# myfavouritekk/vdetlib

Measured on AMD Instinct MI355X. Metric: boxes/sec whole-node (NMS+temporal-conv+link), 300f×10k-box synth; mAP parity, higher is better.
Workload: dtype f32; 1 GPU; configs[1]+[2]: 1 video/GPU, 300 frames x 10000 boxes x 200 classes; per-(frame,class) NMS thresh 0.30 + temporal max-pool w=3 + 3-tap temporal convolution; greedy tubelets: 10 tracks/class (stop < 0.90), IoU-link >= 0.50, spatial max-pool IoU > 0.70 + completion + temporal max-pool; frames=300, boxes=10000, classes=200, scores=rand, parallelism=video-per-gpu x1, 4 distinct videos in flight per GPU

## Files before the change

### vdetlib_amd/csrc/nms_kernels.hpp

```cpp
#pragma once
#include <hip/hip_runtime.h>
#include <stdint.h>

namespace vdet {

struct GroupDesc {
    int32_t box_off;
    int32_t nbox;
    int64_t bits_off;
};

__device__ __host__ __forceinline__ int64_t bit_word(int nbox, int v, int c)
{
    const int W = (nbox + 63) >> 6;
    return ((int64_t)(v >> 6) * W + c) * 64 + (v & 63);
}
__host__ __device__ __forceinline__ int64_t bit_words_of_group(int nbox)
{
    const int64_t W = (nbox + 63) >> 6;
    return W * W * 64;
}

struct TileDesc {
    int32_t group;
// ... 870 lines not shown
        for (int i = tid; i < NW * 256; i += BLOCK) bases[i] = 0;
        __syncthreads();
        uint32_t ra[CPW];
        uint32_t rl[CPW];
        bool peel_on = false;
#pragma unroll
        for (int ch = 0; ch < CPW; ++ch) {
            const int q = (c0 + ch) * 64 + lane;
            const bool valid = (c0 + ch) < nchunks && q < N;
            const uint32_t i = valid ? src[q] : 0u;
            const uint32_t d = valid ? (((uint32_t)keys0[i] >> shift) & 255u) : 0u;
            ra[ch] = i | (d << 16);
            if (ARANK) {
                uint32_t r = 0u;
                bool pending = valid;
#pragma unroll
                for (int peel = 0; peel < 2; ++peel) {
                    if (ch > 0 && !peel_on) break;
                    const unsigned long long rem = __ballot(pending);
                    if (rem) {
                        const int l0 = __ffsll((unsigned long long)rem) - 1;
                        const uint32_t d0 = (uint32_t)__builtin_amdgcn_readlane((int)d, l0);
                        const bool mine = pending && d == d0;
                        const unsigned long long m = __ballot(mine);
                        if (ch == 0 && peel == 0) peel_on = (pass == 3) || __popcll(m) >= 12;
                        if (peel_on) {
                            const uint32_t rank = __builtin_amdgcn_mbcnt_hi((uint32_t)(m >> 32), __builtin_amdgcn_mbcnt_lo((uint32_t)m, 0u));
                            uint32_t old = 0u;
                            if (lane == l0) old = atomicAdd(&bases[w * 256 + d0], (uint32_t)__popcll(m));
                            old = (uint32_t)__builtin_amdgcn_readlane((int)old, l0);
                            if (mine) { r = old + rank; pending = false; }
                        } else {
                            break;
                        }
                    }
                }
                if (pending) r = atomicAdd(&bases[w * 256 + d], 1u);
                rl[ch] = r;
            } else {
                const unsigned long long peers = match8(d, valid);
                const uint32_t rank = __builtin_amdgcn_mbcnt_hi((uint32_t)(peers >> 32), __builtin_amdgcn_mbcnt_lo((uint32_t)peers, 0u));
                uint32_t old = 0;
                if (valid && rank == 0) old = atomicAdd(&bases[w * 256 + d], (uint32_t)__popcll(peers));
                const int leader = valid ? (__ffsll((unsigned long long)peers) - 1) : lane;
                old = __shfl(old, leader, 64);
                rl[ch] = old + rank;
            }
        }
        __syncthreads();
        uint32_t dsum = 0, dincl = 0;
        if (tid < 256) {
#pragma unroll
            for (int ww = 0; ww < NW; ++ww) dsum += bases[ww * 256 + tid];
            dincl = dsum;
#define VDET_SCAN_STEP(CTRL, ROWMASK) dincl += (uint32_t)__builtin_amdgcn_update_dpp(0, (int)dincl, CTRL, ROWMASK, 0xf, false);
            VDET_SCAN_STEP(0x111, 0xf) VDET_SCAN_STEP(0x112, 0xf) VDET_SCAN_STEP(0x114, 0xf) VDET_SCAN_STEP(0x118, 0xf)
            VDET_SCAN_STEP(0x142, 0xa) VDET_SCAN_STEP(0x143, 0xc)
#undef VDET_SCAN_STEP
            if (lane == 63) swt[w] = dincl;
        }
        __syncthreads();
        if (tid < 256) {
            uint32_t run = dincl - dsum;
            for (int k = 0; k < w; ++k) run += swt[k];
#pragma unroll
            for (int ww = 0; ww < NW; ++ww) {
                const uint32_t c = bases[ww * 256 + tid];
                bases[ww * 256 + tid] = run;
                run += c;
            }
        }
        __syncthreads();
#pragma unroll
        for (int ch = 0; ch < CPW; ++ch) {
            const int q = (c0 + ch) * 64 + lane;
            const bool valid = (c0 + ch) < nchunks && q < N;
            if (valid) {
                const uint32_t d = ra[ch] >> 16;
                dst[bases[w * 256 + d] + rl[ch]] = (uint16_t)(ra[ch] & 0xFFFFu);
            }
        }
        __syncthreads();
        uint16_t *t = src; src = dst; dst = t;
    }
    int ncand_out = ncand;
    if (prm.topk > 0 && ncand > prm.topk) {
        const int k = prm.topk;
        if (w == 0) {
            auto key_at = [&](int q) -> uint32_t {
                const int i = src[q];
                if (prm.keys) return prm.keys[pr.sbase + i];
                return score_key(prm.scores[pr.sbase + (int64_t)i * pr.sstride]);
            };
            const uint32_t kk = key_at(k - 1);
            int a = k - 1, b = k;
            for (;;) {
                const int q = a - 1 - lane;
                const bool eq = q >= 0 && key_at(q) == kk;
                const unsigned long long m = __ballot(eq);
                const int n = m == ~0ull ? 64 : (__ffsll((unsigned long long)~m) - 1);
                a -= n;
                if (n < 64) break;
            }
            for (;;) {
                const int q = b + lane;
                const bool eq = q < ncand && key_at(q) == kk;
                const unsigned long long m = __ballot(eq);
                const int n = m == ~0ull ? 64 : (__ffsll((unsigned long long)~m) - 1);
                b += n;
                if (n < 64) break;
            }
            const int nsel = k - a, s0 = b - nsel;
            if (s0 > a)
                for (int t = 0; t < nsel; t += 64) {
                    const bool v = t + lane < nsel;
                    const uint16_t e = v ? src[s0 + t + lane] : (uint16_t)0;
                    __builtin_amdgcn_fence(__ATOMIC_ACQ_REL, "wavefront");
                    if (v) src[a + t + lane] = e;
                    __builtin_amdgcn_fence(__ATOMIC_ACQ_REL, "wavefront");
                }
        }
        ncand_out = k;
        __syncthreads();
    }
    uint16_t *out = prm.order + pr.obase;
    if (((pr.obase | (int64_t)N) & 1) == 0) {
        uint32_t *out2 = reinterpret_cast<uint32_t *>(out);
        const uint32_t *src2 = reinterpret_cast<const uint32_t *>(src);
        for (int v = tid; v < (N >> 1); v += BLOCK) out2[v] = src2[v];
    } else {
        for (int v = tid; v < N; v += BLOCK) out[v] = src[v];
    }
    if (tid == 0) {
        prm.ncand[p] = ncand_out;
        if (prm.nover) prm.nover[p] = ncand;
    }
}

template <int BLOCK, int CPW, bool ARANK>
__global__ __launch_bounds__(BLOCK, (BLOCK == 1024 && CPW <= 10) ? 8 : 1) void sort_kernel(const SortParams prm)
{
    extern __shared__ __attribute__((aligned(16))) unsigned char smem[];
    const int p = xcd_problem(blockIdx.x, gridDim.x);
    if (p >= prm.P) return;
    lsd_sort_problem<BLOCK, CPW, ARANK>(prm, p, smem);
}

template <int BLOCK, int CPW, bool ARANK>
__global__ __launch_bounds__(BLOCK, (BLOCK == 1024 && CPW <= 10) ? 8 : 1) void sort_list_kernel(const SortParams prm, const int32_t *__restrict__ list,
                                                                                                   const int *__restrict__ count)
{
    extern __shared__ __attribute__((aligned(16))) unsigned char smem[];
    const int n = *count;
    for (int i = blockIdx.x; i < n; i += gridDim.x) {
        lsd_sort_problem<BLOCK, CPW, ARANK>(prm, list[i], smem);
        __syncthreads();
    }
}

__global__ __launch_bounds__(64) void lds_atomic_order_probe(const uint8_t *__restrict__ pats, int n, int *__restrict__ bad)
{
    __shared__ uint32_t tbl[256];
    const int lane = threadIdx.x;
    int nbad = 0;
    for (int t = blockIdx.x; t < n; t += gridDim.x) {
        for (int i = lane; i < 256; i += 64) tbl[i] = 0;
        __builtin_amdgcn_fence(__ATOMIC_ACQ_REL, "wavefront");
        const uint32_t d = pats[t * 64 + lane];
        const bool act = d != 255;
        uint32_t r1 = 0, r2 = 0;
        if (act) r1 = atomicAdd(&tbl[d], 1u);
        if (act) r2 = atomicAdd(&tbl[d], 1u);
        const unsigned long long peers = match8(d, act);
        const uint32_t rank = __builtin_amdgcn_mbcnt_hi((uint32_t)(peers >> 32), __builtin_amdgcn_mbcnt_lo((uint32_t)peers, 0u));
        const uint32_t cnt = (uint32_t)__popcll(peers);
        if (act && (r1 != rank || r2 != cnt + rank)) nbad = 1;
        __builtin_amdgcn_fence(__ATOMIC_ACQ_REL, "wavefront");
    }
    if (__ballot(nbad) && lane == 0) atomicOr(bad, 1);
}

__global__ __launch_bounds__(256) void transpose_keys_kernel(const float *__restrict__ scores, uint32_t *__restrict__ keys,
                                                             int B, int C, int use_thr, float thr)
{
    __shared__ uint32_t tile[64][65];
    const int f = blockIdx.z;
    const int b0 = blockIdx.x * 64, c0 = blockIdx.y * 64;
    const int tx = threadIdx.x & 63, ty = threadIdx.x >> 6;
    const float *src = scores + (int64_t)f * B * C;
    for (int r = ty; r < 64; r += 4) {
        const int b = b0 + r, c = c0 + tx;
        uint32_t k = 0;
        if (b < B && c < C) {
            const float s = src[(int64_t)b * C + c];
            k = score_key(s);
            if (use_thr && !(s > thr)) k = 0u;
        }
        tile[r][tx] = k;
    }
    __syncthreads();
    uint32_t *dst = keys + (int64_t)f * C * B;
    for (int r = ty; r < 64; r += 4) {
        const int c = c0 + r, b = b0 + tx;
        if (c < C && b < B) dst[(int64_t)c * B + b] = tile[tx][r];
    }
}

struct WalkParams {
    int mode, P, B, C;
    const GroupDesc *groups;
    const uint16_t *order;
    const int32_t *ncand;
    const uint2 *row_meta;
    const uint16_t *adj;
    const uint32_t *group_z;
    int32_t *keep_idx;
    int32_t *keep_cnt;
    int64_t cap;
    int *status;
    int mask_words;
    const uint32_t *group_flags;
    int wave_words;
    int packed;
    const WalkMeta *wmeta;
    float t32;
    int adj32;
    const uint4 *wmeta16;
};

typedef __attribute__((address_space(3))) uint32_t lds_u32_t;
typedef volatile lds_u32_t *lds_mask_t;

__device__ __forceinline__ lds_mask_t lds_mask_ptr(unsigned char *dyn_smem, int word_off)
{
    return (lds_mask_t)((__attribute__((address_space(3))) unsigned char *)dyn_smem) + word_off;
}
__device__ __forceinline__ void lds_or(lds_mask_t m, int word, uint32_t bits)
{
    __hip_atomic_fetch_or((lds_u32_t *)(m + word), bits, __ATOMIC_RELAXED, __HIP_MEMORY_SCOPE_WAVEFRONT);
}
__device__ __forceinline__ void lds_and(lds_mask_t m, int word, uint32_t bits)
{
    __hip_atomic_fetch_and((lds_u32_t *)(m + word), bits, __ATOMIC_RELAXED, __HIP_MEMORY_SCOPE_WAVEFRONT);
}

__device__ __forceinline__ void lds_or_pair(lds_mask_t m, uint32_t d)
{
    uint32_t w0, w1;
    asm("v_bfe_u32 %0, %1, 5, 11" : "=v"(w0) : "v"(d));
    asm("v_bfe_u32 %0, %1, 21, 11" : "=v"(w1) : "v"(d));
    lds_or(m, (int)w0, 1u << (d & 31u));
    lds_or(m, (int)w1, 1u << ((d >> 16) & 31u));
}

constexpr int kWalkGrp = 4;

template <bool HASZ>
__device__ __forceinline__ void walk_apply_slice(lds_mask_t mask, uint16_t e, bool in_range, int &bad)
{
    if (HASZ) {
        if (in_range) {
            const int v = e & 0x7FFF;
            if (e & kZTag) { if (!((mask[v >> 5] >> (v & 31)) & 1u)) bad = 1; }
            else lds_or(mask, v >> 5, 1u << (v & 31));
        }
    } else {
        if (in_range) lds_or(mask, e >> 5, 1u << (e & 31));
    }
}

template <bool HASZ>
__device__ __forceinline__ void walk_group(lds_mask_t mask, const uint16_t *__restrict__ adj, int lane, int c,
                                           uint32_t off, int deg, const int (&ls)[kWalkGrp], int ng,
                                           const uint32_t (&pre)[kWalkGrp], unsigned long long &kept_lanes, int &bad)
{
#pragma unroll
    for (int k = 0; k < kWalkGrp; ++k) {
        if (k >= ng) break;
        const int cu = __builtin_amdgcn_readlane(c, ls[k]);
        if (__builtin_amdgcn_readfirstlane((mask[cu >> 5] >> (cu & 31)) & 1u)) continue;
        kept_lanes |= 1ull << ls[k];
        const int d = __builtin_amdgcn_readlane(deg, ls[k]);
        if (HASZ && lane == 0) lds_or(mask, cu >> 5, 1u << (cu & 31));
        if (2 * lane < d) {
            walk_apply_slice<HASZ>(mask, (uint16_t)(pre[k] & 0xFFFFu), true, bad);
            walk_apply_slice<HASZ>(mask, (uint16_t)(pre[k] >> 16), true, bad);
        }
        if (d > 128) {
            const uint32_t o = __builtin_amdgcn_readlane(off, ls[k]);
            for (int e0 = 128; e0 < d; e0 += 64)
                walk_apply_slice<HASZ>(mask, adj[o + min(e0 + lane, d - 1)], e0 + lane < d, bad);
        }
    }
}


constexpr int kPackRing = 72;
struct __attribute__((aligned(16))) AdjVec { uint32_t v[4]; };
typedef float lds_f4v __attribute__((ext_vector_type(4)));
typedef volatile __attribute__((address_space(3))) lds_f4v *lds_f4_t;

__device__ __forceinline__ int ring_wrap(int s) { return s >= kPackRing ? s - kPackRing : s; }

__device__ __forceinline__ void walk_ring_drain(const WalkParams &prm, lds_mask_t mask, lds_mask_t ring, lds_f4_t ringb, const int lane,
                                                const float t32, const bool flush, int &qh, int &qn, int &nk,
                                                int32_t *__restrict__ out, const int64_t cap)
{
    const int k = lane >> 3, sub = lane & 7;
    while (qn >= 8 || (flush && qn > 0)) {
        const int ng = min(8, qn);
        const int s = ring_wrap(qh + k);
        const bool vk = k < ng;
        const int sj = ring_wrap(qh + sub);
        const lds_f4v mi = ringb[2 * s];
        const int cm = vk ? (int)__float_as_uint(mi.x) : 0;
        const lds_f4v vi = ringb[2 * s + 1], vj = ringb[2 * sj + 1];
        const float4 bi = make_float4(vi.x, vi.y, vi.z, vi.w), bj = make_float4(vj.x, vj.y, vj.z, vj.w);
        const bool live = vk && !((mask[cm >> 5] >> (cm & 31)) & 1u);
        const unsigned long long lm = __ballot(live);
        const float ai = mi.w, aj = __uint_as_float(ring[8 * sj + 3]);
        bool border;
        bool hit = pred_regular(bi, ai, bj, aj, t32, t32 * 4.76837158203125e-7f, border);
        if (__ballot(border) != 0ull) {
            if (border) hit = (pair_pred(bi, ai, bj, aj, t32) & 1u) != 0u;
        }
        const unsigned long long cmask = __ballot(hit && k < sub && sub < ng && live && ((lm >> (8 * sub)) & 1ull));
        unsigned long long surv_s = lm & 0x0101010101010101ull;
        if (cmask) {
            unsigned long long sv = 0ull;
            for (int j = 0; j < 8; ++j) {
                const unsigned long long col = (cmask >> j) & 0x0101010101010101ull;
                if (((lm >> (8 * j)) & 1ull) && !(col & sv)) sv |= 1ull << (8 * j);
            }
            surv_s = sv;
        }
        const bool surv = (surv_s >> (lane & 56)) & 1ull;
        if (surv_s) {
            const int pos = nk + (int)__builtin_amdgcn_mbcnt_hi((uint32_t)(surv_s >> 32),
                                                               __builtin_amdgcn_mbcnt_lo((uint32_t)surv_s, 0u));
            if (surv && sub == 0 && (int64_t)pos < cap) out[(uint32_t)pos] = cm;
            nk += __popcll(surv_s);
            const uint32_t off = surv ? __float_as_uint(mi.y) : 0u;
            const int deg = surv ? (int)__float_as_uint(mi.z) : 0;
            AdjVec a0, a1;
            if (prm.adj32) {
                const uint32_t bo = off * 2u;
                const char *ab = reinterpret_cast<const char *>(prm.adj);
                a0 = *reinterpret_cast<const AdjVec *>(ab + (bo + (8 * sub < deg ? 16u * (uint32_t)sub : 0u)));
                a1 = *reinterpret_cast<const AdjVec *>(ab + (bo + (64 + 8 * sub < deg ? 128u + 16u * (uint32_t)sub : 0u)));
            } else {
                const AdjVec *pa = reinterpret_cast<const AdjVec *>(prm.adj + off);
                a0 = pa[8 * sub < deg ? sub : 0];
                a1 = pa[64 + 8 * sub < deg ? 8 + sub : 0];
            }
            const bool has0 = 8 * sub < deg, has1 = 64 + 8 * sub < deg;
            if (has0) {
#pragma unroll
                for (int t = 0; t < 4; ++t) {
                    const uint32_t d = a0.v[t];
                    lds_or_pair(mask, d);
                }
            }
            if (__ballot(has1) != 0ull) {
                if (has1) {
#pragma unroll
                    for (int t = 0; t < 4; ++t) {
                        const uint32_t d = a1.v[t];
                        lds_or_pair(mask, d);
                    }
                }
                unsigned long long lg = __ballot(sub == 0 && deg > 128);
                while (lg) {
                    const int l = __ffsll((unsigned long long)lg) - 1;
                    lg &= lg - 1;
                    const uint32_t o = __builtin_amdgcn_readlane(off, l);
                    const int dl = __builtin_amdgcn_readlane(deg, l);
                    for (int e0 = 128; e0 < dl; e0 += 64) {
                        const uint32_t e = prm.adj[o + min(e0 + lane, dl - 1)];
                        if (e0 + lane < dl) lds_or(mask, (int)(e >> 5), 1u << (e & 31u));
                    }
                }
            }
            __builtin_amdgcn_s_waitcnt(0x0F70);
        }
        qh = ring_wrap(qh + ng);
        qn -= ng;
    }
}

template <bool U16>
__device__ __forceinline__ void walk_list_packed(const WalkParams &prm, lds_mask_t mask, const int lane, const int rb,
                                                 const uint16_t *__restrict__ order, const int ncand,
                                                 int32_t *__restrict__ out, const int64_t cap, int &nk_out)
{
    lds_mask_t ring = mask + prm.mask_words;
    lds_f4_t ringb = (lds_f4_t)ring;
    const WalkMeta *__restrict__ wmeta = prm.wmeta + rb;
    const uint4 *__restrict__ wm16 = U16 ? prm.wmeta16 + rb : nullptr;
    const float t32 = prm.t32;
    int qh = 0, qn = 0, nk = 0;
    const int last = max(ncand - 1, 0);
    int cc[3];
    uint2 mm[3];
    float4 bb[3];
    uint4 rr[3];
    cc[0] = (int)order[(uint32_t)min(lane, last)];
    cc[1] = (int)order[(uint32_t)min(64 + lane, last)];
    cc[2] = 0;
    mm[0] = mm[1] = mm[2] = make_uint2(0u, 0u);
    bb[0] = bb[1] = bb[2] = make_float4(0.f, 0.f, 0.f, 0.f);
    rr[0] = rr[1] = rr[2] = make_uint4(0u, 0u, 0u, 0u);
    if (lane < ncand) {
        if (U16) rr[0] = wm16[(uint32_t)cc[0]];
        else { const WalkMeta *wm = wmeta + (uint32_t)cc[0]; bb[0] = wm->box; const uint4 rw = wm->row; mm[0] = make_uint2(rw.x, rw.y); }
    }
#define VDET_WALK_PASS(Q0, CUR, NXT, NN)                                                                                             \
    {                                                                                                                                \
        const int q0_ = (Q0);                                                                                                        \
        const int c = cc[CUR];                                                                                                       \
        cc[NN] = (int)order[(uint32_t)min(q0_ + 128 + lane, last)];                                                                  \
        {    \
             \
            const bool want = (q0_ + 64 + lane) < ncand && !((mask[cc[NXT] >> 5] >> (cc[NXT] & 31)) & 1u);                           \
            if (U16) rr[NXT] = wm16[want ? (uint32_t)cc[NXT] : 0u];                                                                  \
            else {                                                                                                                   \
                const WalkMeta *wm = wmeta + (want ? (uint32_t)cc[NXT] : 0u);                                                        \
                bb[NXT] = wm->box; const uint4 rw = wm->row; mm[NXT] = make_uint2(rw.x, rw.y);                                       \
            }                                                                                                                        \
        }                                                                                                                            \
        const bool alive = (q0_ + lane) < ncand && !((mask[c >> 5] >> (c & 31)) & 1u);                                               \
        const unsigned long long am = __ballot(alive);                                                                               \
        if (alive) {                                                                                                                 \
            const int s = ring_wrap(qh + qn + (int)__builtin_amdgcn_mbcnt_hi((uint32_t)(am >> 32), __builtin_amdgcn_mbcnt_lo((uint32_t)am, 0u))); \
            ring[8 * s] = (uint32_t)c;                                                                                               \
            lds_f4v bv;                                                                                                              \
            if (U16) {                                                                                                               \
                ring[8 * s + 1] = rr[CUR].z;                                                                                         \
                ring[8 * s + 2] = rr[CUR].w;                                                                                         \
                bv.x = (float)(rr[CUR].x & 0xFFFFu); bv.y = (float)(rr[CUR].x >> 16);                                                \
                bv.z = (float)(rr[CUR].y & 0xFFFFu); bv.w = (float)(rr[CUR].y >> 16);                                                \
            } else {                                                                                                                 \
                ring[8 * s + 1] = mm[CUR].x;                                                                                         \
                ring[8 * s + 2] = mm[CUR].y;                                                                                         \
                bv.x = bb[CUR].x; bv.y = bb[CUR].y; bv.z = bb[CUR].z; bv.w = bb[CUR].w;                                              \
            }                                                                                                                        \
            ringb[2 * s + 1] = bv;                                                                                                   \
            ring[8 * s + 3] = __float_as_uint(box_area(make_float4(bv.x, bv.y, bv.z, bv.w)));                                        \
        }                                                                                                                            \
        qn += __popcll(am);                                                                                                          \
        walk_ring_drain(prm, mask, ring, ringb, lane, t32, q0_ + 64 >= ncand, qh, qn, nk, out, cap);                                 \
    }
    for (int q0 = 0; q0 < ncand; q0 += 192) {
        VDET_WALK_PASS(q0, 0, 1, 2)
        if (q0 + 64 >= ncand) break;
        VDET_WALK_PASS(q0 + 64, 1, 2, 0)
        if (q0 + 128 >= ncand) break;
        VDET_WALK_PASS(q0 + 128, 2, 0, 1)
    }
#undef VDET_WALK_PASS
    nk_out = nk;
}

__device__ __forceinline__ void walk_one(const WalkParams &prm, const int p, unsigned char *smem, const int lane, const int w)
{
    lds_mask_t mask = lds_mask_ptr(smem, w * prm.wave_words);
    const ProblemRef pr = decode_problem(prm.mode, p, prm.B, prm.C, prm.groups);
    const int N = pr.N, rb = pr.rb;
    const uint16_t *order = prm.order + pr.obase;
    const int ncand = prm.ncand[p];
    const bool has_z = prm.group_z[pr.g] != 0;
    const bool regular = !has_z && prm.group_flags && (prm.group_flags[pr.g] & kFlagRegular);
    int32_t *out = prm.keep_idx + (prm.mode == 2 ? (int64_t)rb : (int64_t)p * prm.cap);
    const int64_t cap = prm.mode == 2 ? (int64_t)N : prm.cap;

    for (int i = lane; i < ((N + 31) >> 5); i += 64) mask[i] = 0u;
    __builtin_amdgcn_fence(__ATOMIC_ACQ_REL, "wavefront");
    if (has_z) {
        for (int q = ncand + lane; q < N; q += 64) {
            const int v = order[q];
            lds_or(mask, v >> 5, 1u << (v & 31));
        }
        __builtin_amdgcn_fence(__ATOMIC_ACQ_REL, "wavefront");
    }

    int nk = 0;
    int bad = 0;
    if (regular && prm.packed && N >= 2) {
        if (prm.wmeta16 && (prm.group_flags[pr.g] & kFlagU16)) walk_list_packed<true>(prm, mask, lane, rb, order, ncand, out, cap, nk);
        else walk_list_packed<false>(prm, mask, lane, rb, order, ncand, out, cap, nk);
        if (lane == 0) prm.keep_cnt[p] = nk;
        if ((int64_t)nk > cap && lane == 0) atomicOr(prm.status, kStCap);
        return;
    }
    const uint32_t *adjw = reinterpret_cast<const uint32_t *>(prm.adj);
    const int last = max(ncand - 1, 0);
    int c_cur = (int)order[min(lane, last)];
    int c_nxt = (int)order[min(64 + lane, last)];
    uint2 m_cur = make_uint2(0u, 0u);
    if (lane < ncand) m_cur = prm.row_meta[rb + c_cur];
    for (int q0 = 0; q0 < ncand; q0 += 64) {
        const int q = q0 + lane;
        const bool valid = q < ncand;
        const int c = c_cur;
        const int c_nn = (int)order[min(q0 + 128 + lane, last)];
        uint2 m_nxt = make_uint2(0u, 0u);
        if ((q + 64) < ncand && !((mask[c_nxt >> 5] >> (c_nxt & 31)) & 1u)) m_nxt = prm.row_meta[rb + c_nxt];
        const bool alive = valid && !((mask[c >> 5] >> (c & 31)) & 1u);
        unsigned long long am = __ballot(alive);
        unsigned long long kept_lanes = 0ull;
        const uint32_t off = m_cur.x;
        const int deg = (int)m_cur.y;
        while (am) {
            int ls[kWalkGrp];
            int ng = 0;
#pragma unroll
            for (int k = 0; k < kWalkGrp; ++k) {
                ls[k] = k ? ls[k - 1] : 0;
                if (am) { ls[k] = __builtin_amdgcn_readfirstlane(__ffsll((unsigned long long)am) - 1); am &= am - 1; ng = k + 1; }
            }
            uint32_t pre[kWalkGrp];
#pragma unroll
            for (int k = 0; k < kWalkGrp; ++k) {
                const uint32_t o = __builtin_amdgcn_readlane(off, ls[k]);
                const int d = __builtin_amdgcn_readlane(deg, ls[k]);
                pre[k] = adjw[(o >> 1) + min(lane, (max(d, 1) - 1) >> 1)];
            }
            if (has_z) walk_group<true>(mask, prm.adj, lane, c, off, deg, ls, ng, pre, kept_lanes, bad);
            else walk_group<false>(mask, prm.adj, lane, c, off, deg, ls, ng, pre, kept_lanes, bad);
        }
        if (kept_lanes) {
            const int pos = nk + (int)__builtin_amdgcn_mbcnt_hi((uint32_t)(kept_lanes >> 32),
                                                               __builtin_amdgcn_mbcnt_lo((uint32_t)kept_lanes, 0u));
            if (((kept_lanes >> lane) & 1ull) && (int64_t)pos < cap) out[pos] = c;
            nk += __popcll(kept_lanes);
        }
        c_cur = c_nxt; c_nxt = c_nn; m_cur = m_nxt;
    }
    if (lane == 0) prm.keep_cnt[p] = nk;
    if ((int64_t)nk > cap && lane == 0) atomicOr(prm.status, kStCap);
    if (__ballot(bad != 0) && lane == 0) atomicOr(prm.status, kStDivZero);
}

__global__ __launch_bounds__(256) void walk_kernel(const WalkParams prm)
{
    extern __shared__ __attribute__((aligned(16))) unsigned char smem[];
    const int lane = threadIdx.x & 63, w = __builtin_amdgcn_readfirstlane(threadIdx.x >> 6);
    const int nwaves_total = gridDim.x * 4;
    const int per = nwaves_total >> 3;
    const int p = (blockIdx.x & 7) * per + (blockIdx.x >> 3) * 4 + w;
    if (p >= prm.P) return;
    walk_one(prm, p, smem, lane, w);
}

__global__ __launch_bounds__(256) void check_order_kernel(const uint16_t *__restrict__ order, const int32_t *__restrict__ ncand_in, int P, int B,
                                                          int32_t *__restrict__ ncand_out, int *__restrict__ status)
{
    const int lane = threadIdx.x & 63;
    const int p = blockIdx.x * 4 + (threadIdx.x >> 6);
    if (p >= P) return;
    const int n = ncand_in[p];
    bool bad = n < 0 || n > B;
    if (!bad)
        for (int q = lane; q < n; q += 64) bad = bad || (int)order[(int64_t)p * B + q] >= B;
    const bool any = __ballot(bad) != 0ull;
    if (lane == 0) {
        ncand_out[p] = any ? 0 : n;
        if (any) atomicOr(status, kStBadOrder);
    }
}

__global__ __launch_bounds__(256) void gather_comp_kernel(const GroupDesc *__restrict__ groups, int P,
                                                          const int32_t *__restrict__ keep_idx,
                                                          const int32_t *__restrict__ keep_cnt,
                                                          const float *__restrict__ scores,
                                                          const uint32_t *__restrict__ keys,
                                                          const uint32_t *__restrict__ orig_idx,
                                                          unsigned long long *__restrict__ comp,
                                                          unsigned int *__restrict__ glob_cnt)
{
    __shared__ unsigned int sbase;
    const int p = blockIdx.x;
    if (p >= P) return;
    const int rb = groups[p].box_off;
    const int K = keep_cnt[p];
    if (threadIdx.x == 0) sbase = atomicAdd(glob_cnt, (unsigned int)K);
    __syncthreads();
    const unsigned int base = sbase;
    for (int k = threadIdx.x; k < K; k += 256) {
        const int v = keep_idx[rb + k];
        const uint32_t key = keys ? keys[rb + v] : score_key(scores[rb + v]);
        comp[base + k] = ((unsigned long long)key << 32) | orig_idx[rb + v];
    }
}

__global__ void bitonic_global_step(unsigned long long *__restrict__ data, uint32_t n2, uint32_t j, uint32_t k)
{
    const uint32_t i = blockIdx.x * blockDim.x + threadIdx.x;
    if (i >= n2) return;
    const uint32_t ixj = i ^ j;
    if (ixj > i) {
        const unsigned long long a = data[i], b = data[ixj];
        const bool desc = (i & k) == 0;
        if (desc ? (a < b) : (a > b)) { data[i] = b; data[ixj] = a; }
    }
}

__global__ __launch_bounds__(1024) void bitonic_lds_kernel(unsigned long long *__restrict__ data, uint32_t n2,
                                                           uint32_t k_first, uint32_t k_last)
{
    __shared__ unsigned long long s[2048];
    const uint32_t base = blockIdx.x * 2048u;
    const uint32_t tid = threadIdx.x;
    for (uint32_t i = tid; i < 2048u; i += 1024u) s[i] = (base + i < n2) ? data[base + i] : 0ull;
    __syncthreads();
    for (uint32_t k = k_first; k <= k_last; k <<= 1) {
        uint32_t j0 = k >> 1;
        if (j0 > 1024u) j0 = 1024u;
        for (uint32_t j = j0; j > 0; j >>= 1) {
            for (uint32_t li = tid; li < 2048u; li += 1024u) {
                const uint32_t lixj = li ^ j;
                if (lixj > li) {
                    const uint32_t gi = base + li;
                    const unsigned long long a = s[li], b = s[lixj];
                    const bool desc = (gi & k) == 0;
                    if (desc ? (a < b) : (a > b)) { s[li] = b; s[lixj] = a; }
                }
            }
            __syncthreads();
        }
    }
    for (uint32_t i = tid; i < 2048u; i += 1024u)
        if (base + i < n2) data[base + i] = s[i];
}

__global__ void fill_comp_kernel(const float *__restrict__ scores, const uint32_t *__restrict__ keys,
                                 const uint8_t *__restrict__ excl, int use_thr, float thr, int64_t base, int n,
                                 uint32_t n2, unsigned long long *__restrict__ comp, int32_t *__restrict__ ncand_p)
{
    const uint32_t i = blockIdx.x * blockDim.x + threadIdx.x;
    if (i >= n2) return;
    unsigned long long c = 0ull;
    if ((int)i < n) {
        uint32_t k;
        bool x = false;
        if (keys) { k = keys[base + i]; x = (k == 0u); }
        else {
            const float sc = scores[base + i];
            k = score_key(sc);
            if (use_thr && !(sc > thr)) x = true;
        }
        if (excl && excl[base + i]) x = true;
        if (x) k = 0u; else atomicAdd(ncand_p, 1);
        c = ((unsigned long long)k << 32) | i;
    }
    comp[i] = c;
}

__global__ void comp_to_order_kernel(const unsigned long long *__restrict__ comp, int n, uint16_t *__restrict__ order)
{
    const int i = blockIdx.x * blockDim.x + threadIdx.x;
    if (i < n) order[i] = (uint16_t)(comp[i] & 0xFFFFull);
}

__global__ void comp_to_index_kernel(const unsigned long long *__restrict__ comp, uint32_t n, int64_t *__restrict__ out)
{
    const uint32_t i = blockIdx.x * blockDim.x + threadIdx.x;
    if (i < n) out[i] = (int64_t)(comp[i] & 0xFFFFFFFFull);
}

__global__ void track_round1_kernel(const float *__restrict__ det_frame, const float4 *__restrict__ det_box, int m,
                                    const float *__restrict__ trk_frame, const float4 *__restrict__ trk_box, int t,
                                    float t32, uint8_t *__restrict__ excl, int *__restrict__ status)
{
    const int i = blockIdx.x * blockDim.x + threadIdx.x;
    if (i >= m) return;
    const float4 bi = det_box[i];
    const float iarea = box_area(bi);
    const float fi = det_frame[i];
    uint8_t sup = 0;
    for (int j = 0; j < t; ++j) {
        if (fi != trk_frame[j]) continue;
        const float4 bt = trk_box[j];
        const uint32_t p = pair_pred(bi, iarea, bt, box_area(bt), t32);
        if (p & 2u) { atomicOr(status, kStDivZero); break; }
        if (p & 1u) { sup = 1; break; }
    }
    excl[i] = sup;
}

}
```

Before: 348.2 million boxes/s.

## Software-pipeline adjacency list loads across ring-drain groups in NMS walk

Restructures the NMS walk's ring drain so the adjacency vectors for the next 8-candidate group are requested before the current group's suppression bits are applied. Partial waitcnts then overlap the global-memory latency with the LDS mask OR work. The kept-index write becomes a branchless raw buffer store, with out-of-range offsets used to drop masked lanes. The walk kernel also gets an 8-waves-per-EU occupancy hint. In exchange, adjacency rows are loaded for groups whose candidates may not survive, and the forced occupancy may push the kernel into register spills.

```diff
diff --git a/vdetlib_amd/csrc/nms_kernels.hpp b/vdetlib_amd/csrc/nms_kernels.hpp
--- a/vdetlib_amd/csrc/nms_kernels.hpp
+++ b/vdetlib_amd/csrc/nms_kernels.hpp
@@ -1196,90 +1196,122 @@
 
 __device__ __forceinline__ int ring_wrap(int s) { return s >= kPackRing ? s - kPackRing : s; }
 
+__device__ __forceinline__ void walk_lists_request(const WalkParams &prm, lds_f4_t ringb, const int qh, const int ng, const int k,
+                                                   const int sub, AdjVec &a0, AdjVec &a1)
+{
+    const lds_f4v mi = ringb[2 * ring_wrap(qh + k)];
+    const bool vk = k < ng;
+    const uint32_t off = vk ? __float_as_uint(mi.y) : 0u;
+    const int deg = vk ? (int)__float_as_uint(mi.z) : 0;
+    if (prm.adj32) {
+        const uint32_t bo = off * 2u;
+        const char *ab = reinterpret_cast<const char *>(prm.adj);
+        a0 = *reinterpret_cast<const AdjVec *>(ab + (bo + (8 * sub < deg ? 16u * (uint32_t)sub : 0u)));
+        a1 = *reinterpret_cast<const AdjVec *>(ab + (bo + (64 + 8 * sub < deg ? 128u + 16u * (uint32_t)sub : 0u)));
+    } else {
+        const AdjVec *pa = reinterpret_cast<const AdjVec *>(prm.adj + off);
+        a0 = pa[8 * sub < deg ? sub : 0];
+        a1 = pa[64 + 8 * sub < deg ? 8 + sub : 0];
+    }
+}
+
+__device__ __forceinline__ unsigned long long walk_group_survivors(lds_mask_t mask, lds_mask_t ring, lds_f4_t ringb, const int qh, const int ng,
+                                                                   const int k, const int sub, const float t32, int &cm, uint32_t &off, int &deg)
+{
+    const int s = ring_wrap(qh + k);
+    const bool vk = k < ng;
+    const int sj = ring_wrap(qh + sub);
+    const lds_f4v mi = ringb[2 * s];
+    cm = vk ? (int)__float_as_uint(mi.x) : 0;
+    off = __float_as_uint(mi.y);
+    deg = (int)__float_as_uint(mi.z);
+    const lds_f4v vi = ringb[2 * s + 1], vj = ringb[2 * sj + 1];
+    const float4 bi = make_float4(vi.x, vi.y, vi.z, vi.w), bj = make_float4(vj.x, vj.y, vj.z, vj.w);
+    const bool live = vk && !((mask[cm >> 5] >> (cm & 31)) & 1u);
+    const unsigned long long lm = __ballot(live);
+    const float ai = mi.w, aj = __uint_as_float(ring[8 * sj + 3]);
+    bool border;
+    bool hit = pred_regular(bi, ai, bj, aj, t32, t32 * 4.76837158203125e-7f, border);
+    if (__ballot(border) != 0ull) {
+        if (border) hit = (pair_pred(bi, ai, bj, aj, t32) & 1u) != 0u;
+    }
+    const unsigned long long cmask = __ballot(hit && k < sub && sub < ng && live && ((lm >> (8 * sub)) & 1ull));
+    unsigned long long surv_s = lm & 0x0101010101010101ull;
+    if (cmask) {
+        unsigned long long sv = 0ull;
+        for (int j = 0; j < 8; ++j) {
+            const unsigned long long col = (cmask >> j) & 0x0101010101010101ull;
+            if (((lm >> (8 * j)) & 1ull) && !(col & sv)) sv |= 1ull << (8 * j);
+        }
+        surv_s = sv;
+    }
+    return surv_s;
+}
+
+__device__ __forceinline__ void walk_lists_apply(const WalkParams &prm, lds_mask_t mask, const int lane, const int sub, const bool surv,
+                                                 const uint32_t off, const int deg, const AdjVec &a0, const AdjVec &a1)
+{
+    const bool has0 = surv && 8 * sub < deg, has1 = surv && 64 + 8 * sub < deg;
+    if (has0) {
+#pragma unroll
+        for (int t = 0; t < 4; ++t) {
+            const uint32_t d = a0.v[t];
+            lds_or_pair(mask, d);
+        }
+    }
+    if (__ballot(has1) != 0ull) {
+        if (has1) {
+#pragma unroll
+            for (int t = 0; t < 4; ++t) {
+                const uint32_t d = a1.v[t];
+                lds_or_pair(mask, d);
+            }
+        }
+        unsigned long long lg = __ballot(surv && sub == 0 && deg > 128);
+        while (lg) {
+            const int l = __ffsll((unsigned long long)lg) - 1;
+            lg &= lg - 1;
+            const uint32_t o = __builtin_amdgcn_readlane(off, l);
+            const int dl = __builtin_amdgcn_readlane(deg, l);
+            for (int e0 = 128; e0 < dl; e0 += 64) {
+                const uint32_t e = prm.adj[o + min(e0 + lane, dl - 1)];
+                if (e0 + lane < dl) lds_or(mask, (int)(e >> 5), 1u << (e & 31u));
+            }
+        }
+    }
+}
+
 __device__ __forceinline__ void walk_ring_drain(const WalkParams &prm, lds_mask_t mask, lds_mask_t ring, lds_f4_t ringb, const int lane,
                                                 const float t32, const bool flush, int &qh, int &qn, int &nk,
-                                                int32_t *__restrict__ out, const int64_t cap)
+                                                const __amdgpu_buffer_rsrc_t outr, const int64_t cap)
 {
     const int k = lane >> 3, sub = lane & 7;
-    while (qn >= 8 || (flush && qn > 0)) {
+    auto turn = [&](const AdjVec &c0, const AdjVec &c1, AdjVec &n0, AdjVec &n1) __attribute__((always_inline)) -> bool {
         const int ng = min(8, qn);
-        const int s = ring_wrap(qh + k);
-        const bool vk = k < ng;
-        const int sj = ring_wrap(qh + sub);
-        const lds_f4v mi = ringb[2 * s];
-        const int cm = vk ? (int)__float_as_uint(mi.x) : 0;
-        const lds_f4v vi = ringb[2 * s + 1], vj = ringb[2 * sj + 1];
-        const float4 bi = make_float4(vi.x, vi.y, vi.z, vi.w), bj = make_float4(vj.x, vj.y, vj.z, vj.w);
-        const bool live = vk && !((mask[cm >> 5] >> (cm & 31)) & 1u);
-        const unsigned long long lm = __ballot(live);
-        const float ai = mi.w, aj = __uint_as_float(ring[8 * sj + 3]);
-        bool border;
-        bool hit = pred_regular(bi, ai, bj, aj, t32, t32 * 4.76837158203125e-7f, border);
-        if (__ballot(border) != 0ull) {
-            if (border) hit = (pair_pred(bi, ai, bj, aj, t32) & 1u) != 0u;
-        }
-        const unsigned long long cmask = __ballot(hit && k < sub && sub < ng && live && ((lm >> (8 * sub)) & 1ull));
-        unsigned long long surv_s = lm & 0x0101010101010101ull;
-        if (cmask) {
-            unsigned long long sv = 0ull;
-            for (int j = 0; j < 8; ++j) {
-                const unsigned long long col = (cmask >> j) & 0x0101010101010101ull;
-                if (((lm >> (8 * j)) & 1ull) && !(col & sv)) sv |= 1ull << (8 * j);
-            }
-            surv_s = sv;
-        }
+        int cm, deg;
+        uint32_t off;
+        const unsigned long long surv_s = walk_group_survivors(mask, ring, ringb, qh, ng, k, sub, t32, cm, off, deg);
         const bool surv = (surv_s >> (lane & 56)) & 1ull;
-        if (surv_s) {
-            const int pos = nk + (int)__builtin_amdgcn_mbcnt_hi((uint32_t)(surv_s >> 32),
-                                                               __builtin_amdgcn_mbcnt_lo((uint32_t)surv_s, 0u));
-            if (surv && sub == 0 && (int64_t)pos < cap) out[(uint32_t)pos] = cm;
-            nk += __popcll(surv_s);
-            const uint32_t off = surv ? __float_as_uint(mi.y) : 0u;
-            const int deg = surv ? (int)__float_as_uint(mi.z) : 0;
-            AdjVec a0, a1;
-            if (prm.adj32) {
-                const uint32_t bo = off * 2u;
-                const char *ab = reinterpret_cast<const char *>(prm.adj);
-                a0 = *reinterpret_cast<const AdjVec *>(ab + (bo + (8 * sub < deg ? 16u * (uint32_t)sub : 0u)));
-                a1 = *reinterpret_cast<const AdjVec *>(ab + (bo + (64 + 8 * sub < deg ? 128u + 16u * (uint32_t)sub : 0u)));
-            } else {
-                const AdjVec *pa = reinterpret_cast<const AdjVec *>(prm.adj + off);
-                a0 = pa[8 * sub < deg ? sub : 0];
-                a1 = pa[64 + 8 * sub < deg ? 8 + sub : 0];
-            }
-            const bool has0 = 8 * sub < deg, has1 = 64 + 8 * sub < deg;
-            if (has0) {
-#pragma unroll
-                for (int t = 0; t < 4; ++t) {
-                    const uint32_t d = a0.v[t];
-                    lds_or_pair(mask, d);
-                }
-            }
-            if (__ballot(has1) != 0ull) {
-                if (has1) {
-#pragma unroll
-                    for (int t = 0; t < 4; ++t) {
-                        const uint32_t d = a1.v[t];
-                        lds_or_pair(mask, d);
-                    }
-                }
-                unsigned long long lg = __ballot(sub == 0 && deg > 128);
-                while (lg) {
-                    const int l = __ffsll((unsigned long long)lg) - 1;
-                    lg &= lg - 1;
-                    const uint32_t o = __builtin_amdgcn_readlane(off, l);
-                    const int dl = __builtin_amdgcn_readlane(deg, l);
-                    for (int e0 = 128; e0 < dl; e0 += 64) {
-                        const uint32_t e = prm.adj[o + min(e0 + lane, dl - 1)];
-                        if (e0 + lane < dl) lds_or(mask, (int)(e >> 5), 1u << (e & 31u));
-                    }
-                }
-            }
-            __builtin_amdgcn_s_waitcnt(0x0F70);
-        }
+        const int pos = nk + (int)__builtin_amdgcn_mbcnt_hi((uint32_t)(surv_s >> 32), __builtin_amdgcn_mbcnt_lo((uint32_t)surv_s, 0u));
+        __builtin_amdgcn_raw_buffer_store_b32(cm, outr, (surv && sub == 0 && (int64_t)pos < cap) ? (uint32_t)pos * 4u : 0x80000000u, 0, 0);
+        nk += __popcll(surv_s);
         qh = ring_wrap(qh + ng);
         qn -= ng;
-    }
+        const bool more = qn >= 8 || (flush && qn > 0);
+        if (more) {
+            walk_lists_request(prm, ringb, qh, min(8, qn), k, sub, n0, n1);
+            __builtin_amdgcn_s_waitcnt(0x0F73);
+            walk_lists_apply(prm, mask, lane, sub, surv, off, deg, c0, c1);
+            return true;
+        }
+        __builtin_amdgcn_s_waitcnt(0x0F71);
+        walk_lists_apply(prm, mask, lane, sub, surv, off, deg, c0, c1);
+        return false;
+    };
+    if (!(qn >= 8 || (flush && qn > 0))) return;
+    AdjVec a0, a1, b0, b1;
+    walk_lists_request(prm, ringb, qh, min(8, qn), k, sub, a0, a1);
+    while (turn(a0, a1, b0, b1) && turn(b0, b1, a0, a1)) { }
 }
 
 template <bool U16>
@@ -1293,6 +1325,7 @@
     const uint4 *__restrict__ wm16 = U16 ? prm.wmeta16 + rb : nullptr;
     const float t32 = prm.t32;
     int qh = 0, qn = 0, nk = 0;
+    const __amdgpu_buffer_rsrc_t outr = __builtin_amdgcn_make_buffer_rsrc((void *)out, (short)0, (int)(min(cap, (int64_t)0x10000) * 4), 0x00020000);
     const int last = max(ncand - 1, 0);
     int cc[3];
     uint2 mm[3];
@@ -1342,7 +1375,7 @@
             ring[8 * s + 3] = __float_as_uint(box_area(make_float4(bv.x, bv.y, bv.z, bv.w)));                                        \
         }                                                                                                                            \
         qn += __popcll(am);                                                                                                          \
-        walk_ring_drain(prm, mask, ring, ringb, lane, t32, q0_ + 64 >= ncand, qh, qn, nk, out, cap);                                 \
+        walk_ring_drain(prm, mask, ring, ringb, lane, t32, q0_ + 64 >= ncand, qh, qn, nk, outr, cap);                                          \
     }
     for (int q0 = 0; q0 < ncand; q0 += 192) {
         VDET_WALK_PASS(q0, 0, 1, 2)
@@ -1435,7 +1468,7 @@
     if (__ballot(bad != 0) && lane == 0) atomicOr(prm.status, kStDivZero);
 }
 
-__global__ __launch_bounds__(256) void walk_kernel(const WalkParams prm)
+__global__ __launch_bounds__(256) __attribute__((amdgpu_waves_per_eu(8, 8))) void walk_kernel(const WalkParams prm)
 {
     extern __shared__ __attribute__((aligned(16))) unsigned char smem[];
     const int lane = threadIdx.x & 63, w = __builtin_amdgcn_readfirstlane(threadIdx.x >> 6);
```

Result: no change. 346.7 million boxes/s (-0.4%).
